# Qixiaomao/video-caption-algorithm

Hardware: AMD Instinct MI355X
Metric: captions/sec + p50 encode+decode latency, 16-frame ViT-B/16 → GPT-2-small, 1/2/4/8 GPU (higher is better)
Workload: dtype bf16

## Files before the change

video-caption-algorithm_amd/csrc/gemm256.hip:

```cpp
#include <cstdlib>

#include "vcap_common.h"
#include "vcap_kernels.h"

namespace {

constexpr int TM = 256, TN = 256, ROWB = 128;
constexpr int HALF = 128 * ROWB;
constexpr int BUF = 4 * HALF;
constexpr int LDS_BYTES = 2 * BUF;
constexpr int SBUF = 2048;
constexpr int LDS_BYTES_MX = LDS_BYTES + 4 * SBUF;

VCAP_DEV void glds16(const void* g, char* lds_wave_base) {
  __builtin_amdgcn_global_load_lds((const __attribute__((address_space(1))) void*)g,
                                   (__attribute__((address_space(3))) void*)lds_wave_base, 16, 0, 0);
}

template <typename T, int GS>
VCAP_DEV void half_offsets(uint32_t (&off)[2], long ld, int rows, int base, int X, int wave, int lane) {
  constexpr int E = Frag<T>::kElems;
#pragma unroll
  for (int i = 0; i < 2; ++i) {
    const int lr = (wave * 2 + i) * 8 + (lane >> 3);
    const int c = (lane & 7) ^ (lr & 7);
    int gr = base + (lr >> GS) * (2 << GS) + X * (1 << GS) + (lr & ((1 << GS) - 1));
    gr = gr < rows ? gr : rows - 1;
    off[i] = (uint32_t)(((long)gr * ld + c * E) * (long)sizeof(T));
  }
}

VCAP_DEV void glds4(const void* g, char* lds_wave_base) {
  __builtin_amdgcn_global_load_lds((const __attribute__((address_space(1))) void*)g,
                                   (__attribute__((address_space(3))) void*)lds_wave_base, 4, 0, 0);
}

VCAP_DEV void stage_half(const char* base_k, const uint32_t (&off)[2], char* lds_half, int wave) {
#pragma unroll
  for (int i = 0; i < 2; ++i) glds16(base_k + off[i], lds_half + (wave * 2 + i) * 1024);
}

VCAP_DEV u32x4 frag(const char* half, int row, int chunk) {
  return *reinterpret_cast<const u32x4*>(half + row * ROWB + ((chunk ^ (row & 7)) << 4));
}

template <typename V>
VCAP_DEV void out_store(V* p, const V& v) {
  if constexpr (__is_same(V, f32x4)) *p = v;
  else __builtin_nontemporal_store(v, p);
}

template <typename TOut>
VCAP_DEV uint32_t pack_out2(float lo, float hi) {
  if constexpr (sizeof(TOut) == 2) return Pack2<TOut>::pack(lo, hi);
  else return 0u;
}

VCAP_DEV void lds_fence() { asm volatile("" ::: "memory"); }

}


template <typename TIn, typename TOut, int EPI>
VCAP_DEV void epilogue256(const f32x4 (&acc)[2][2][4][2], int m0, int n0, int wr, int wc, int lane, int M, int N,
                          TOut* C, long ldc, const GemmEpi& epi) {
  const int fr = lane & 15, fg = lane >> 4;
  if constexpr (EPI == 4) {
    uint64_t sc[2] = {0, 0};
    f32x4 biasq[2][2];
#pragma unroll
    for (int qn = 0; qn < 2; ++qn)
#pragma unroll
      for (int j = 0; j < 2; ++j)
        biasq[qn][j] = *reinterpret_cast<const f32x4*>(epi.bias + min(n0 + wc * 64 + qn * 32 + j * 16 + fg * 4, N - 4));
#pragma unroll
    for (int qm = 0; qm < 2; ++qm)
#pragma unroll
      for (int i = 0; i < 4; i += 2) {
        uint32_t x[2][4];
#pragma unroll
        for (int qn = 0; qn < 2; ++qn)
#pragma unroll
          for (int h = 0; h < 2; ++h) {
            f32x4 v[2];
            float amax = 0.f;
#pragma unroll
            for (int j = 0; j < 2; ++j) {
              v[j] = gelu_tanh4(acc[qm][qn][i + h][j] + biasq[qn][j]);
#pragma unroll
              for (int e = 0; e < 4; ++e) amax = fmaxf(amax, fabsf(v[j][e]));
            }
            amax = rows_max(amax);
            const int sbyte = mx_scale_byte(amax);
            const float inv = mx_inv_scale(sbyte);
            const f32x4 q0 = v[0] * inv, q1 = v[1] * inv;
            x[qn][2 * h] = pack_fp8x4(q0.x, q0.y, q0.z, q0.w);
            x[qn][2 * h + 1] = pack_fp8x4(q1.x, q1.y, q1.z, q1.w);
            sc[qn] |= (uint64_t)(uint32_t)sbyte << (8 * (qm * 4 + i + h));
          }
        const int nb0 = n0 + wc * 64;
#pragma unroll
        for (int h = 0; h < 2; ++h) {
          uint32_t y[4] = {x[0][2 * h], x[0][2 * h + 1], x[1][2 * h], x[1][2 * h + 1]};
          transpose4_groups(y);
          const int ms = m0 + wr * 128 + qm * 64 + (i + h) * 16 + fr;
          if (ms < M && nb0 < N)
            out_store(reinterpret_cast<u32x4*>((uint8_t*)C + (long)ms * ldc + nb0 + fg * 16),
                      (u32x4){y[0], y[1], y[2], y[3]});
        }
      }
#pragma unroll
    for (int qn = 0; qn < 2; ++qn) {
      const int nb = n0 + wc * 64 + qn * 32;
      if (fg == 0 && nb < N)
        *reinterpret_cast<uint64_t*>(epi.c_scale + mx_scale_index(m0 + wr * 128 + fr, nb, (M + 255) >> 8)) = sc[qn];
    }
  } else if (sizeof(TOut) == 2 && (EPI == 0 || EPI == 1) && (N & 31) == 0 && (ldc & 7) == 0 &&
             ((uintptr_t)C & 15) == 0) {
    const bool odd = (lane & 16) != 0;
#pragma unroll
    for (int qm = 0; qm < 2; ++qm)
#pragma unroll
      for (int qn = 0; qn < 2; ++qn) {
        const int nb = n0 + wc * 64 + qn * 32;
        f32x4 bias[2];
#pragma unroll
        for (int j = 0; j < 2; ++j)
          bias[j] = epi.bias ? *reinterpret_cast<const f32x4*>(epi.bias + min(nb + j * 16 + fg * 4, N - 4))
                             : (f32x4){0.f, 0.f, 0.f, 0.f};
        const int col = nb + (odd ? 12 + 4 * fg : 4 * fg);
#pragma unroll
        for (int i = 0; i < 4; ++i) {
          const int m = m0 + wr * 128 + qm * 64 + i * 16 + fr;
          uint32_t p[2][2];
#pragma unroll
          for (int j = 0; j < 2; ++j) {
            f32x4 v = acc[qm][qn][i][j] + bias[j];
            if constexpr (EPI == 1) v = gelu_tanh4(Autocast<TIn>::rnd4(v));
            p[j][0] = pack_out2<TOut>(v.x, v.y);
            p[j][1] = pack_out2<TOut>(v.z, v.w);
          }
          const uint32_t r0 = (uint32_t)xor16_i((int)(odd ? p[0][0] : p[1][0]));
          const uint32_t r1 = (uint32_t)xor16_i((int)(odd ? p[0][1] : p[1][1]));
          const u32x4 o = odd ? (u32x4){r0, r1, p[1][0], p[1][1]} : (u32x4){p[0][0], p[0][1], r0, r1};
          if (m < M && nb < N) out_store(reinterpret_cast<u32x4*>(C + (long)m * ldc + col), o);
        }
      }
  } else if constexpr (EPI == 2) {
    f32x4 bias[2][2];
#pragma unroll
    for (int qn = 0; qn < 2; ++qn)
#pragma unroll
      for (int j = 0; j < 2; ++j) {
        const int n = min(n0 + wc * 64 + qn * 32 + j * 16 + fg * 4, N - 4);
        bias[qn][j] = epi.bias ? *reinterpret_cast<const f32x4*>(epi.bias + n) : (f32x4){0.f, 0.f, 0.f, 0.f};
      }
    auto res_load = [&](f32x4 (&r)[4][2], int qm, int qn) {
#pragma unroll
      for (int i = 0; i < 4; ++i)
#pragma unroll
        for (int j = 0; j < 2; ++j) {
          const int m = min(m0 + wr * 128 + qm * 64 + i * 16 + fr, M - 1);
          const int n = min(n0 + wc * 64 + qn * 32 + j * 16 + fg * 4, N - 4);
          r[i][j] = *reinterpret_cast<const f32x4*>(epi.res + (long)m * epi.ldr + n);
        }
    };
    auto res_store = [&](const f32x4 (&r)[4][2], int qm, int qn) {
#pragma unroll
      for (int i = 0; i < 4; ++i)
#pragma unroll
        for (int j = 0; j < 2; ++j) {
          const int m = m0 + wr * 128 + qm * 64 + i * 16 + fr;
          const int n = n0 + wc * 64 + qn * 32 + j * 16 + fg * 4;
          const f32x4 v = Autocast<TIn>::rnd4(acc[qm][qn][i][j] + bias[qn][j]) + r[i][j];
          if (m < M && n < N) out_store(reinterpret_cast<f32x4*>(C + (long)m * ldc + n), v);
        }
    };
    f32x4 r0[4][2], r1[4][2];
    res_load(r0, 0, 0);
    res_load(r1, 0, 1);
    res_store(r0, 0, 0);
    res_load(r0, 1, 0);
    res_store(r1, 0, 1);
    res_load(r1, 1, 1);
    res_store(r0, 1, 0);
    res_store(r1, 1, 1);
  } else {
#pragma unroll
  for (int qm = 0; qm < 2; ++qm)
#pragma unroll
    for (int qn = 0; qn < 2; ++qn)
#pragma unroll
      for (int j = 0; j < 2; ++j) {
        const int n = n0 + wc * 64 + qn * 32 + j * 16 + fg * 4;
        if (n >= N) continue;
        const f32x4 bias = epi.bias ? *reinterpret_cast<const f32x4*>(epi.bias + n) : (f32x4){0.f, 0.f, 0.f, 0.f};
#pragma unroll
        for (int i = 0; i < 4; ++i) {
          const int m = m0 + wr * 128 + qm * 64 + i * 16 + fr;
          if (m >= M) continue;
          f32x4 v = acc[qm][qn][i][j] + bias;
          if constexpr (!(EPI == 0 && sizeof(TOut) == 2)) v = Autocast<TIn>::rnd4(v);
          long orow = m;
          if constexpr (EPI == 1) {
#pragma unroll
            for (int e = 0; e < 4; ++e) v[e] = gelu_tanh(v[e]);
          } else if constexpr (EPI == 2) {
            v += *reinterpret_cast<const f32x4*>(epi.res + orow * epi.ldr + n);
          } else if constexpr (EPI == 3) {
            if (epi.act == 1)
#pragma unroll
              for (int e = 0; e < 4; ++e) v[e] = sizeof(TOut) == 4 ? Autocast<TIn>::rnd(gelu_tanh(v[e])) : gelu_tanh(v[e]);
            orow = epi.G ? (long)(m / epi.G) * epi.Gs + epi.goff + (m % epi.G) : (long)m;
            if (epi.res_mode == 1) v += *reinterpret_cast<const f32x4*>(epi.res + orow * epi.ldr + n);
            else if (epi.res_mode == 2)
              v += *reinterpret_cast<const f32x4*>(epi.res + (long)((m % epi.G) + epi.roff) * epi.ldr + n);
          }
          if constexpr (sizeof(TOut) == 2) {
            out_store(reinterpret_cast<u32x2*>(C + orow * ldc + n),
                      (u32x2){Pack2<TOut>::pack(v.x, v.y), Pack2<TOut>::pack(v.z, v.w)});
          } else {
            out_store(reinterpret_cast<f32x4*>(C + orow * ldc + n), v);
          }
        }
      }
  }
}

template <typename TIn, typename TOut, int EPI>
__global__ __launch_bounds__(512) void vcap_gemm256_kernel(const TIn* __restrict__ A, long lda,
                                                           const TIn* __restrict__ W, long ldw, TOut* C, long ldc,
                                                           int M, int N, int K, GemmEpi epi) {
  extern __shared__ __attribute__((aligned(16))) char smem[];
  constexpr int BK = ROWB / sizeof(TIn);
  constexpr bool MX = sizeof(TIn) == 1;

  const int tiles_n = (N + TN - 1) / TN;
  const int tiles_m = (M + TM - 1) / TM;
  const int nwg = tiles_m * tiles_n;
  const int bid = blockIdx.x;
  const int xcd = bid & 7, q = nwg >> 3, r8 = nwg & 7;
  const int wgid = (xcd < r8 ? xcd * (q + 1) : r8 * (q + 1) + (xcd - r8) * q) + (bid >> 3);
  int mt, nt;
  if (epi.colgroup > 0) {
    const int w = epi.colgroup, per = w * tiles_m;
    const int g = wgid / per, rem = wgid - g * per;
    mt = rem / w;
    nt = g * w + (rem - (rem / w) * w);
  } else {
    mt = wgid / tiles_n;
    nt = wgid - mt * tiles_n;
  }
  const int m0 = mt * TM, n0 = nt * TN;

  const int tid = threadIdx.x, lane = tid & 63;
  const int wave = __builtin_amdgcn_readfirstlane(tid >> 6);
  const int wr = wave >> 2, wc = wave & 3;
  const int fr = lane & 15, fg = lane >> 4;

  f32x4 acc[2][2][4][2];
#pragma unroll
  for (int a = 0; a < 2; ++a)
#pragma unroll
    for (int b = 0; b < 2; ++b)
#pragma unroll
      for (int i = 0; i < 4; ++i)
#pragma unroll
        for (int j = 0; j < 2; ++j) acc[a][b][i][j] = (f32x4){0.f, 0.f, 0.f, 0.f};
  u32x8 a0[4], a1[4], b0[2], b1[2];
  int sa[2], sb;

  uint32_t offA[2][2], offB[2][2];
  half_offsets<TIn, 6>(offA[0], lda, M, m0, 0, wave, lane);
  half_offsets<TIn, 6>(offA[1], lda, M, m0, 1, wave, lane);
  half_offsets<TIn, 5>(offB[0], ldw, N, n0, 0, wave, lane);
  half_offsets<TIn, 5>(offB[1], ldw, N, n0, 1, wave, lane);
  const uint8_t* s_src = nullptr;
  long s_stride = 0;
  if constexpr (MX) {
    const int ga = (M + 255) >> 8, gw = (N + 255) >> 8;
    s_src = wave < 4 ? epi.a_scale + (long)(m0 >> 8) * 1024 : epi.w_scale + (long)(n0 >> 8) * 1024;
    s_src += (wave & 3) * 256;
    s_stride = (long)(wave < 4 ? ga : gw) * 1024;
  }
  char* const sbase = smem + 2 * BUF;
  auto stA = [&](int X, int kt) {
    stage_half((const char*)A + (long)kt * ROWB, offA[X], smem + (kt & 1) * BUF + X * HALF, wave);
    if constexpr (MX) {
      if (X == 0) glds4(s_src + kt * s_stride + lane * 4, sbase + (kt & 3) * SBUF + wave * 256);
    }
  };
  auto stB = [&](int Y, int kt) {
    stage_half((const char*)W + (long)kt * ROWB, offB[Y], smem + (kt & 1) * BUF + (2 + Y) * HALF, wave);
  };
  auto rdA = [&](u32x8 (&f)[4], int X, int kt) {
    const char* h = smem + (kt & 1) * BUF + X * HALF;
#pragma unroll
    for (int i = 0; i < 4; ++i) {
      const int row = wr * 64 + i * 16 + fr;
      f[i] = cat8(frag(h, row, fg), frag(h, row, 4 + fg));
    }
  };
  auto rdB = [&](u32x8 (&f)[2], int Y, int kt) {
    const char* h = smem + (kt & 1) * BUF + (2 + Y) * HALF;
#pragma unroll
    for (int j = 0; j < 2; ++j) {
      const int row = wc * 32 + j * 16 + fr;
      f[j] = cat8(frag(h, row, fg), frag(h, row, 4 + fg));
    }
  };
  auto rdS = [&](int kt) {
    if constexpr (MX) {
      const char* sb_ = sbase + (kt & 3) * SBUF + fg * 256 + fr * 16;
      const u32x2 a = *reinterpret_cast<const u32x2*>(sb_ + wr * 8);
      sa[0] = (int)a.x;
      sa[1] = (int)a.y;
      sb = (int)*reinterpret_cast<const uint32_t*>(sb_ + 1024 + wc * 4);
    }
  };
  auto mma = [&](f32x4 (&c)[4][2], const u32x8 (&af)[4], int X, const u32x8 (&bf)[2], int Y) {
    __builtin_amdgcn_s_setprio(1);
    if constexpr (MX) {
      const int s_a = sa[X];
      asm volatile("s_nop 1" ::: "memory");
#define VCAP_MX4(YY)                                           \
      mfma_mx<YY * 2 + 0, 0>(bf[0], sb, af[0], s_a, c[0][0]);  \
      mfma_mx<YY * 2 + 1, 0>(bf[1], sb, af[0], s_a, c[0][1]);  \
      mfma_mx<YY * 2 + 0, 1>(bf[0], sb, af[1], s_a, c[1][0]);  \
      mfma_mx<YY * 2 + 1, 1>(bf[1], sb, af[1], s_a, c[1][1]);  \
      mfma_mx<YY * 2 + 0, 2>(bf[0], sb, af[2], s_a, c[2][0]);  \
      mfma_mx<YY * 2 + 1, 2>(bf[1], sb, af[2], s_a, c[2][1]);  \
      mfma_mx<YY * 2 + 0, 3>(bf[0], sb, af[3], s_a, c[3][0]);  \
      mfma_mx<YY * 2 + 1, 3>(bf[1], sb, af[3], s_a, c[3][1]);
      if (Y == 0) {
        VCAP_MX4(0)
      } else {
        VCAP_MX4(1)
      }
#undef VCAP_MX4
    } else {
#pragma unroll
      for (int i = 0; i < 4; ++i)
#pragma unroll
        for (int j = 0; j < 2; ++j) c[i][j] = mfma_frag(lo4(bf[j]), lo4(af[i]), c[i][j], (TIn*)nullptr);
#pragma unroll
      for (int i = 0; i < 4; ++i)
#pragma unroll
        for (int j = 0; j < 2; ++j) c[i][j] = mfma_frag(hi4(bf[j]), hi4(af[i]), c[i][j], (TIn*)nullptr);
    }
    __builtin_amdgcn_s_setprio(0);
  };
  auto wait_landed = [&]() {
    if constexpr (MX) asm volatile("s_waitcnt vmcnt(7)" ::: "memory");
    else asm volatile("s_waitcnt vmcnt(6)" ::: "memory");
  };
  auto sync_reads = [&]() {
    asm volatile("s_waitcnt lgkmcnt(0)" ::: "memory");
    lds_fence();
    __builtin_amdgcn_s_barrier();
  };
  auto end_phase = [&]() {
    lds_fence();
    __builtin_amdgcn_s_barrier();
    lds_fence();
  };

  const int nk = K / BK;
  stA(0, 0);
  stA(1, 0);
  stB(0, 0);
  stB(1, 0);
  stA(0, 1);
  stB(0, 1);
  stB(1, 1);
  wait_landed();
  end_phase();
  if (wr == 1) __builtin_amdgcn_s_barrier();

  for (int t = 0; t < nk; t += 2) {
    const bool more = t + 2 < nk;
    rdB(b0, 0, t);
    rdA(a0, 0, t);
    rdS(t);
    stA(1, t + 1);
    sync_reads();
    mma(acc[0][0], a0, 0, b0, 0);
    end_phase();

    rdB(b1, 1, t);
    if (more) stA(0, t + 2);
    sync_reads();
    mma(acc[0][1], a0, 0, b1, 1);
    end_phase();

    rdA(a1, 1, t);
    if (more) stB(0, t + 2);
    sync_reads();
    mma(acc[1][1], a1, 1, b1, 1);
    end_phase();

    if (more) {
      stB(1, t + 2);
      wait_landed();
    } else {
      asm volatile("s_waitcnt vmcnt(0)" ::: "memory");
    }
    sync_reads();
    mma(acc[1][0], a1, 1, b0, 0);
    end_phase();

    rdB(b0, 0, t + 1);
    rdA(a0, 0, t + 1);
    rdS(t + 1);
    if (more) stA(1, t + 2);
    sync_reads();
    mma(acc[0][0], a0, 0, b0, 0);
    end_phase();

    rdB(b1, 1, t + 1);
    if (more) stA(0, t + 3);
    sync_reads();
    mma(acc[0][1], a0, 0, b1, 1);
    end_phase();

    rdA(a1, 1, t + 1);
    if (more) stB(0, t + 3);
    sync_reads();
    mma(acc[1][1], a1, 1, b1, 1);
    end_phase();

    if (more) {
      stB(1, t + 3);
      wait_landed();
    }
    sync_reads();
    mma(acc[1][0], a1, 1, b0, 0);
    end_phase();
  }
  if (wr == 0) __builtin_amdgcn_s_barrier();
  if constexpr (MX) mfma_mx_drain();

  epilogue256<TIn, TOut, EPI>(acc, m0, n0, wr, wc, lane, M, N, C, ldc, epi);
}

template <typename TIn, typename TOut, int EPI>
static hipError_t launch256_epi(const void* A, long lda, const void* W, long ldw, void* C, long ldc, int M, int N,
                                int K, const GemmEpi& epi, hipStream_t s) {
  constexpr int lds = sizeof(TIn) == 1 ? LDS_BYTES_MX : LDS_BYTES;
  static bool configured = false;
  if (!configured) {
    hipError_t e = hipFuncSetAttribute((const void*)vcap_gemm256_kernel<TIn, TOut, EPI>,
                                       hipFuncAttributeMaxDynamicSharedMemorySize, lds);
    if (e != hipSuccess) return e;
    configured = true;
  }
  const int tiles_n = (N + TN - 1) / TN;
  const int tiles = ((M + TM - 1) / TM) * tiles_n;
  GemmEpi e = epi;
  e.colgroup = 0;
  if (EPI == 1) {
    const long tile_bytes = (long)TN * K * (long)sizeof(TIn);
    int w = 0;
    for (int c = tiles_n - 1; c >= 1; --c)
      if (tiles_n % c == 0 && c * tile_bytes <= 2560L * 1024) {
        w = c;
        break;
      }
    if (w > 0 && w < tiles_n && tiles_n % w == 0) e.colgroup = w;
  }
  hipLaunchKernelGGL((vcap_gemm256_kernel<TIn, TOut, EPI>), dim3(tiles), dim3(512), lds, s, (const TIn*)A, lda,
                     (const TIn*)W, ldw, (TOut*)C, ldc, M, N, K, e);
  return hipGetLastError();
}

template <typename TIn, typename TOut>
static hipError_t launch256(const void* A, long lda, const void* W, long ldw, void* C, long ldc, int M, int N, int K,
                            const GemmEpi& epi, hipStream_t s) {
  if constexpr (sizeof(TOut) == 1) {
    return launch256_epi<TIn, TOut, 4>(A, lda, W, ldw, C, ldc, M, N, K, epi, s);
  } else {
    const bool plain_rows = epi.G == 0;
    if (plain_rows && epi.res_mode == 0 && epi.act == 0)
      return launch256_epi<TIn, TOut, 0>(A, lda, W, ldw, C, ldc, M, N, K, epi, s);
    if constexpr (sizeof(TOut) == sizeof(TIn) || sizeof(TOut) == 2) {
      if (plain_rows && epi.res_mode == 0 && epi.act == 1)
        return launch256_epi<TIn, TOut, 1>(A, lda, W, ldw, C, ldc, M, N, K, epi, s);
    }
    if constexpr (sizeof(TOut) == 4) {
      if (plain_rows && epi.res_mode == 1 && epi.act == 0 && epi.res == (const float*)C && epi.ldr == ldc)
        return launch256_epi<TIn, TOut, 2>(A, lda, W, ldw, C, ldc, M, N, K, epi, s);
    }
    return launch256_epi<TIn, TOut, 3>(A, lda, W, ldw, C, ldc, M, N, K, epi, s);
  }
}

bool vcap_gemm256_ok(int in_dt, int out_dt, long lda, long ldw, long ldc, int M, int N, int K, const GemmEpi& epi) {
  if (!vcap_dt_size(in_dt) || !vcap_dt_size(out_dt)) return false;
  const int bk = 128 / (int)vcap_dt_size(in_dt);
  if (K % (2 * bk) != 0 || N % 16 != 0 || M <= 0) return false;
  const int ein = 16 / (int)vcap_dt_size(in_dt);
  if (in_dt == VCAP_DT_MXFP8 && (!epi.a_scale || !epi.w_scale)) return false;
  if (out_dt == VCAP_DT_MXFP8 && (in_dt != VCAP_DT_MXFP8 || N % 128 || ldc % 16 || epi.act != 1 || !epi.bias ||
                                  !epi.c_scale || epi.G || epi.res_mode))
    return false;
  if (lda % ein || ldw % ein) return false;
  if (ldc % 4) return false;
  if (epi.bias && ((uintptr_t)epi.bias & 15)) return false;
  if (epi.res && (((uintptr_t)epi.res & 15) || epi.ldr % 4)) return false;
  (void)out_dt;
  return true;
}

hipError_t vcap_gemm256_dispatch(int in_dt, int out_dt, const void* A, long lda, const void* W, long ldw, void* C,
                                 long ldc, int M, int N, int K, const GemmEpi& epi, hipStream_t s) {
  if (in_dt == VCAP_DT_BF16 && out_dt == VCAP_DT_BF16)
    return launch256<bf16_t, bf16_t>(A, lda, W, ldw, C, ldc, M, N, K, epi, s);
  if (in_dt == VCAP_DT_BF16 && out_dt == VCAP_DT_F32)
    return launch256<bf16_t, float>(A, lda, W, ldw, C, ldc, M, N, K, epi, s);
  if (in_dt == VCAP_DT_F16 && out_dt == VCAP_DT_F16)
    return launch256<f16_t, f16_t>(A, lda, W, ldw, C, ldc, M, N, K, epi, s);
  if (in_dt == VCAP_DT_F16 && out_dt == VCAP_DT_F32)
    return launch256<f16_t, float>(A, lda, W, ldw, C, ldc, M, N, K, epi, s);
  if (in_dt == VCAP_DT_F32 && out_dt == VCAP_DT_F32)
    return launch256<float, float>(A, lda, W, ldw, C, ldc, M, N, K, epi, s);
  if (in_dt == VCAP_DT_MXFP8 && out_dt == VCAP_DT_BF16)
    return launch256<fp8_t, bf16_t>(A, lda, W, ldw, C, ldc, M, N, K, epi, s);
  if (in_dt == VCAP_DT_MXFP8 && out_dt == VCAP_DT_F32)
    return launch256<fp8_t, float>(A, lda, W, ldw, C, ldc, M, N, K, epi, s);
  if (in_dt == VCAP_DT_MXFP8 && out_dt == VCAP_DT_MXFP8)
    return launch256<fp8_t, fp8_t>(A, lda, W, ldw, C, ldc, M, N, K, epi, s);
  return hipErrorInvalidValue;
}
```

Before: 1306.

## Prefetch residual tile into LDS during final K iterations of gemm256

For the in-place fp32 residual-add epilogue (EPI 2, bf16 input), the kernel now issues global-to-LDS loads of the residual tile during the last K-loop iteration, reusing freed staging buffers plus a small extra LDS region. The remaining pieces are loaded into registers. The epilogue then reads the residual from LDS and registers instead of fetching it from global memory after the loop. The aim is to hide residual load latency behind the final MFMAs, at the cost of more LDS per block (possibly lower occupancy), tighter vmcnt bookkeeping, and extra register pressure.

```diff
diff --git a/video-caption-algorithm_amd/csrc/gemm256.hip b/video-caption-algorithm_amd/csrc/gemm256.hip
--- a/video-caption-algorithm_amd/csrc/gemm256.hip
+++ b/video-caption-algorithm_amd/csrc/gemm256.hip
@@ -35,7 +35,9 @@
                                    (__attribute__((address_space(3))) void*)lds_wave_base, 4, 0, 0);
 }
 
+template <bool PIN = false>
 VCAP_DEV void stage_half(const char* base_k, const uint32_t (&off)[2], char* lds_half, int wave) {
+  if constexpr (PIN) asm volatile("" : "+s"(base_k));
 #pragma unroll
   for (int i = 0; i < 2; ++i) glds16(base_k + off[i], lds_half + (wave * 2 + i) * 1024);
 }
@@ -57,6 +59,56 @@
 }
 
 VCAP_DEV void lds_fence() { asm volatile("" ::: "memory"); }
+VCAP_DEV int lane_id() { return (int)__builtin_amdgcn_mbcnt_hi(~0u, __builtin_amdgcn_mbcnt_lo(~0u, 0u)); }
+
+template <typename TIn, int EPI>
+constexpr bool kResPrefetch = EPI == 2 && sizeof(TIn) == 2;
+struct ResPieces {
+  static constexpr int kSpare = 4, kLds = 16 + kSpare, kReg = 32 - kLds;
+  static constexpr int kLdsBytes = LDS_BYTES + 8 * kSpare * 1024;
+};
+
+VCAP_DEV char* res_piece_lds(char* smem, int p, int wave) {
+  using R = ResPieces;
+  if (p >= 8 && p < 8 + R::kSpare) return smem + LDS_BYTES + (wave * R::kSpare + p - 8) * 1024;
+  const int q = p < 8 ? p : p - 8 - R::kSpare;
+  const int s = q >> 1;
+  const int h = s == 0 ? 0 : s == 3 ? 1 : s + 1;
+  return smem + (p < 8 ? 0 : BUF) + h * HALF + (wave * 2 + (q & 1)) * 1024;
+}
+
+VCAP_DEV bool res_prefetch_tile(int m0, int n0, int M, int N) { return m0 + TM <= M && n0 + TN <= N; }
+VCAP_DEV const char* res_wave_base(const GemmEpi& epi, int m0, int n0, int wr, int wc) {
+  return reinterpret_cast<const char*>(epi.res + (long)(m0 + wr * 128) * epi.ldr + n0 + wc * 64);
+}
+VCAP_DEV long res_piece_off(int p, long ldr) {
+  return ((long)((p >> 4) * 64 + ((p >> 1) & 3) * 16) * ldr + ((p >> 3) & 1) * 32 + (p & 1) * 16) * 4;
+}
+VCAP_DEV uint32_t res_lane_off(int lane, long ldr) { return (uint32_t)((lane & 15) * (int)ldr + (lane >> 4) * 4) * 4u; }
+constexpr long kResMaxLd = 1L << 24;
+
+struct ResStage {
+  char* smem;
+  const char* base;
+  long ldr;
+  uint32_t lo;
+  int wave;
+  bool on;
+  VCAP_DEV void operator()(int p0, int p1) const {
+    if (!on) return;
+    const char* b = base;
+    asm volatile("" : "+s"(b));
+#pragma unroll
+    for (int p = p0; p < p1; ++p) glds16(b + res_piece_off(p, ldr) + lo, res_piece_lds(smem, p, wave));
+  }
+};
+
+template <int N>
+VCAP_DEV void wait_vm_seen() {
+  lds_fence();
+  __builtin_amdgcn_s_waitcnt((N & 15) | ((N >> 4) << 14) | (7 << 4) | (15 << 8));
+  lds_fence();
+}
 
 }
 
@@ -227,6 +279,40 @@
   }
 }
 
+template <typename TIn>
+VCAP_DEV void epilogue256_prefetched(const f32x4 (&acc)[2][2][4][2], const char* smem, int m0, int n0, int wr, int wc,
+                                     int wave, int lane, uint32_t lo, float* C, long ldc, const GemmEpi& epi) {
+  using R = ResPieces;
+  const char* rbase = res_wave_base(epi, m0, n0, wr, wc);
+  const float* bsrc = (epi.bias ? epi.bias : epi.res) + n0 + wc * 64 + (lane >> 4) * 4;
+  f32x4 bias[2][2], rr[R::kReg];
+#pragma unroll
+  for (int qn = 0; qn < 2; ++qn)
+#pragma unroll
+    for (int j = 0; j < 2; ++j) bias[qn][j] = *reinterpret_cast<const f32x4*>(bsrc + qn * 32 + j * 16);
+#pragma unroll
+  for (int k = 0; k < R::kReg; ++k)
+    rr[k] = *reinterpret_cast<const f32x4*>(rbase + res_piece_off(R::kLds + k, epi.ldr) + lo);
+  wait_vm_seen<R::kReg>();
+  if (!epi.bias) {
+#pragma unroll
+    for (int qn = 0; qn < 2; ++qn)
+#pragma unroll
+      for (int j = 0; j < 2; ++j) bias[qn][j] = (f32x4){0.f, 0.f, 0.f, 0.f};
+  }
+  float* cw = C + (long)(m0 + wr * 128 + (lane & 15)) * ldc + n0 + wc * 64 + (lane >> 4) * 4;
+  auto store = [&](int p, const f32x4& r) {
+    const int qm = p >> 4, qn = (p >> 3) & 1, i = (p >> 1) & 3, j = p & 1;
+    const f32x4 v = Autocast<TIn>::rnd4(acc[qm][qn][i][j] + bias[qn][j]) + r;
+    out_store(reinterpret_cast<f32x4*>(cw + (long)(qm * 64 + i * 16) * ldc + qn * 32 + j * 16), v);
+  };
+#pragma unroll
+  for (int p = 0; p < R::kLds; ++p)
+    store(p, *reinterpret_cast<const f32x4*>(res_piece_lds(const_cast<char*>(smem), p, wave) + lane * 16));
+#pragma unroll
+  for (int k = 0; k < R::kReg; ++k) store(R::kLds + k, rr[k]);
+}
+
 template <typename TIn, typename TOut, int EPI>
 __global__ __launch_bounds__(512) void vcap_gemm256_kernel(const TIn* __restrict__ A, long lda,
                                                            const TIn* __restrict__ W, long ldw, TOut* C, long ldc,
@@ -234,6 +320,7 @@
   extern __shared__ __attribute__((aligned(16))) char smem[];
   constexpr int BK = ROWB / sizeof(TIn);
   constexpr bool MX = sizeof(TIn) == 1;
+  constexpr bool PF = kResPrefetch<TIn, EPI>;
 
   const int tiles_n = (N + TN - 1) / TN;
   const int tiles_m = (M + TM - 1) / TM;
@@ -285,13 +372,13 @@
   }
   char* const sbase = smem + 2 * BUF;
   auto stA = [&](int X, int kt) {
-    stage_half((const char*)A + (long)kt * ROWB, offA[X], smem + (kt & 1) * BUF + X * HALF, wave);
+    stage_half<PF>((const char*)A + (long)kt * ROWB, offA[X], smem + (kt & 1) * BUF + X * HALF, wave);
     if constexpr (MX) {
       if (X == 0) glds4(s_src + kt * s_stride + lane * 4, sbase + (kt & 3) * SBUF + wave * 256);
     }
   };
   auto stB = [&](int Y, int kt) {
-    stage_half((const char*)W + (long)kt * ROWB, offB[Y], smem + (kt & 1) * BUF + (2 + Y) * HALF, wave);
+    stage_half<PF>((const char*)W + (long)kt * ROWB, offB[Y], smem + (kt & 1) * BUF + (2 + Y) * HALF, wave);
   };
   auto rdA = [&](u32x8 (&f)[4], int X, int kt) {
     const char* h = smem + (kt & 1) * BUF + X * HALF;
@@ -366,6 +453,11 @@
   };
 
   const int nk = K / BK;
+  constexpr int XS = ResPieces::kSpare;
+  ResStage stR{};
+  if constexpr (PF)
+    stR = ResStage{smem, res_wave_base(epi, m0, n0, wr, wc), epi.ldr, res_lane_off(lane, epi.ldr), wave,
+                   res_prefetch_tile(m0, n0, M, N)};
   stA(0, 0);
   stA(1, 0);
   stB(0, 0);
@@ -383,18 +475,23 @@
     rdA(a0, 0, t);
     rdS(t);
     stA(1, t + 1);
+    if constexpr (PF) {
+      if (!more) stR(8, 8 + XS);
+    }
     sync_reads();
     mma(acc[0][0], a0, 0, b0, 0);
     end_phase();
 
     rdB(b1, 1, t);
     if (more) stA(0, t + 2);
+    else if constexpr (PF) stR(0, 2);
     sync_reads();
     mma(acc[0][1], a0, 0, b1, 1);
     end_phase();
 
     rdA(a1, 1, t);
     if (more) stB(0, t + 2);
+    else if constexpr (PF) stR(2, 4);
     sync_reads();
     mma(acc[1][1], a1, 1, b1, 1);
     end_phase();
@@ -402,6 +499,9 @@
     if (more) {
       stB(1, t + 2);
       wait_landed();
+    } else if (stR.on) {
+      stR(4, 6);
+      wait_vm_seen<XS + 6>();
     } else {
       asm volatile("s_waitcnt vmcnt(0)" ::: "memory");
     }
@@ -413,18 +513,21 @@
     rdA(a0, 0, t + 1);
     rdS(t + 1);
     if (more) stA(1, t + 2);
+    else if constexpr (PF) stR(6, 8);
     sync_reads();
     mma(acc[0][0], a0, 0, b0, 0);
     end_phase();
 
     rdB(b1, 1, t + 1);
     if (more) stA(0, t + 3);
+    else if constexpr (PF) stR(8 + XS, 12 + XS);
     sync_reads();
     mma(acc[0][1], a0, 0, b1, 1);
     end_phase();
 
     rdA(a1, 1, t + 1);
     if (more) stB(0, t + 3);
+    else if constexpr (PF) stR(12 + XS, 14 + XS);
     sync_reads();
     mma(acc[1][1], a1, 1, b1, 1);
     end_phase();
@@ -432,6 +535,8 @@
     if (more) {
       stB(1, t + 3);
       wait_landed();
+    } else if constexpr (PF) {
+      stR(14 + XS, 16 + XS);
     }
     sync_reads();
     mma(acc[1][0], a1, 1, b0, 0);
@@ -440,13 +545,19 @@
   if (wr == 0) __builtin_amdgcn_s_barrier();
   if constexpr (MX) mfma_mx_drain();
 
-  epilogue256<TIn, TOut, EPI>(acc, m0, n0, wr, wc, lane, M, N, C, ldc, epi);
+  if constexpr (PF) {
+    if (stR.on) epilogue256_prefetched<TIn>(acc, smem, m0, n0, wr, wc, wave, lane_id(), stR.lo, C, ldc, epi);
+    else epilogue256<TIn, TOut, EPI>(acc, m0, n0, wr, wc, lane_id(), M, N, C, ldc, epi);
+  } else {
+    epilogue256<TIn, TOut, EPI>(acc, m0, n0, wr, wc, lane, M, N, C, ldc, epi);
+  }
 }
 
 template <typename TIn, typename TOut, int EPI>
 static hipError_t launch256_epi(const void* A, long lda, const void* W, long ldw, void* C, long ldc, int M, int N,
                                 int K, const GemmEpi& epi, hipStream_t s) {
-  constexpr int lds = sizeof(TIn) == 1 ? LDS_BYTES_MX : LDS_BYTES;
+  constexpr bool MX = sizeof(TIn) == 1;
+  constexpr int lds = kResPrefetch<TIn, EPI> ? ResPieces::kLdsBytes : MX ? LDS_BYTES_MX : LDS_BYTES;
   static bool configured = false;
   if (!configured) {
     hipError_t e = hipFuncSetAttribute((const void*)vcap_gemm256_kernel<TIn, TOut, EPI>,
@@ -487,7 +598,8 @@
         return launch256_epi<TIn, TOut, 1>(A, lda, W, ldw, C, ldc, M, N, K, epi, s);
     }
     if constexpr (sizeof(TOut) == 4) {
-      if (plain_rows && epi.res_mode == 1 && epi.act == 0 && epi.res == (const float*)C && epi.ldr == ldc)
+      if (plain_rows && epi.res_mode == 1 && epi.act == 0 && epi.res == (const float*)C && epi.ldr == ldc &&
+          epi.ldr < kResMaxLd)
         return launch256_epi<TIn, TOut, 2>(A, lda, W, ldw, C, ldc, M, N, K, epi, s);
     }
     return launch256_epi<TIn, TOut, 3>(A, lda, W, ldw, C, ldc, M, N, K, epi, s);
```

After: 1328, median of 6. 1.02x the previous value.
